# researchaccelerator-hub/distributed-crawler

Measured on AMD Instinct MI355X. Metric: posts/sec (whole node) synthetic feed, higher is better.
Workload: dtype uint8; 1 GPU; model=telegram-crawl 1k-channels x 10k-posts per GPU (BASELINE config #2, weak-scaled), global_batch=1250000, seq_len=0, platform=telegram, parallelism=dp1, channels_per_gpu=1000, posts_per_channel=10000, chunk_posts=1250000, new_discoveries=998486, sink=pinned, pinned=True, max_comments_per_post=3

## Files before the change

crawler_amd/ops/csrc/common.h:

```cpp
#pragma once

#include <hip/hip_runtime.h>
#include <stdint.h>

#define WAVE 64
#define DEV __device__ __forceinline__

typedef unsigned int __attribute__((aligned(1))) u32_unal;
#ifndef CRAWL_NT_STORES
#define CRAWL_NT_STORES 0
#endif
DEV void nt_store_u32(unsigned char* p, unsigned v) {
#if CRAWL_NT_STORES
  __builtin_nontemporal_store(v, (u32_unal*)p);
#else
  __builtin_memcpy(p, &v, 4);
#endif
}
DEV void nt_store_u8(unsigned char* p, unsigned char v) {
#if CRAWL_NT_STORES
  __builtin_nontemporal_store(v, p);
#else
  *p = v;
#endif
}

namespace crawl {

DEV int lane_id() { return threadIdx.x & (WAVE - 1); }
DEV int wave_id() { return threadIdx.x >> 6; }

// ... 220 lines not shown
  DEV void raw(const uint8_t* s, int n) {
    if (W) {
      int lane = lane_id();
      int nw = n >> 2;
      for (int k = lane; k < nw; k += WAVE) {
        unsigned w;
        __builtin_memcpy(&w, s + 4 * k, 4);
        nt_store_u32(out + cur + 4 * k, w);
      }
      for (int j = (nw << 2) + lane; j < n; j += WAVE)
        nt_store_u8(out + cur + j, s[j]);
    }
    cur += n;
  }

  static DEV bool swar_special(unsigned w) {
    unsigned hz;
    unsigned nonascii = w & 0x80808080u;
    unsigned lt20 = (w - 0x20202020u) & ~w & 0x80808080u;
    if (lt20) return true;
    hz = ((w ^ 0x22222222u) - 0x01010101u) & ~(w ^ 0x22222222u);
    hz |= ((w ^ 0x5C5C5C5Cu) - 0x01010101u) & ~(w ^ 0x5C5C5C5Cu);
    hz |= ((w ^ 0x3C3C3C3Cu) - 0x01010101u) & ~(w ^ 0x3C3C3C3Cu);
    hz |= ((w ^ 0x3E3E3E3Eu) - 0x01010101u) & ~(w ^ 0x3E3E3E3Eu);
    hz |= ((w ^ 0x26262626u) - 0x01010101u) & ~(w ^ 0x26262626u);
    if (hz & 0x80808080u) return true;
    if (nonascii) {
      unsigned e2 = ((w ^ 0xE2E2E2E2u) - 0x01010101u) & ~(w ^ 0xE2E2E2E2u);
      if (e2 & 0x80808080u) return true;
    }
// ... 62 lines not shown
        unsigned d;
        if (v <= 0xFFFFFFFFULL)
          d = ((unsigned)v / (unsigned)POW10[lane]) % 10u;
        else
          d = (unsigned)((v / POW10[lane]) % 10ULL);
        nt_store_u8(out + cur + n - 1 - lane, (uint8_t)('0' + d));
      }
    }
    cur += n;
  }
  DEV void i64(long long v) {
    if (v < 0) { LIT(*this, "-"); u64((unsigned long long)(-v)); }
    else u64((unsigned long long)v);
  }

  DEV void rfc3339(long long secs) {
    if (W) rfc3339_write(out, cur, secs);
    cur += 20;
  }
};

DEV uint64_t fnv1a64(const uint8_t* s, int n) {
  uint64_t h = 1469598103934665603ULL;
  for (int i = 0; i < n; ++i) {
    h ^= s[i];
    h *= 1099511628211ULL;
  }
  return h;
}

// ... 2 lines not shown
```

crawler_amd/ops/csrc/parse_encode.hip:

```cpp

#include "common.h"
#include "tg_lits.h"

namespace crawl {

#define MAX_LINKS 8
#define TG_STAGE_BYTES 3968

struct BatchView {
  const long* __restrict__ chat_id;
  const long* __restrict__ msg_id;
  const long* __restrict__ text_off;
  const int* __restrict__ date;
  const int* __restrict__ content_type;
  const int* __restrict__ views;
  const int* __restrict__ forwards;
  const int* __restrict__ media_album_id;
  const int* __restrict__ channel_idx;
  const int* __restrict__ flags;
  const int* __restrict__ text_len;
  const int* __restrict__ aux_off;
  const int* __restrict__ aux_len;
  const int* __restrict__ ent_off;
  const int* __restrict__ ent_cnt;
// ... 24 lines not shown
  const int* __restrict__ ch_title_off;
  const int* __restrict__ ch_title_len;
  const unsigned char* __restrict__ emoji_pool;
  const int* __restrict__ emoji_off;
  const int* __restrict__ emoji_len;
  const unsigned char* __restrict__ created_str;
  int created_len;
  const unsigned char* __restrict__ capture_str;
  int capture_len;
  int n;
  int skip_media;
  long min_post_date;
  const unsigned char* __restrict__ ctname_pool;
  const int* __restrict__ ctname_off;
  const int* __restrict__ ctname_len;
};

struct LinkOut {
  unsigned char* __restrict__ name;
  unsigned char* __restrict__ name_len;
  unsigned char* __restrict__ src;
  int* __restrict__ cnt;
  unsigned long long* __restrict__ hash;
};


DEV void utf16_to_bytes(const unsigned char* s, int n, int off16, int len16,
                        int* out_start, int* out_end) {
  int lane = lane_id();
  int run = 0;
// ... 174 lines not shown
    LIT(*this, "\"");
  }
};

struct StagedTabs {
  const unsigned char* emoji_pool;
  const int* emoji_off;
  const int* emoji_len;
  const unsigned char* created;
  const unsigned char* capture;
  const unsigned char* ctname_pool;
  const int* ctname_off;
  const int* ctname_len;
};

template <bool W, bool STAGED>
DEV int emit_line(const BatchView& B, int i, unsigned char* out,
                  LinkList& L, const unsigned char* lds_lits,
                  unsigned char* lds_stage, const StagedTabs* T) {
  const int lane = lane_id();
  Emit<W> e{};
  e.out = out;
  e.cur = 0;
  e.lds = lds_lits;
  const int c = B.channel_idx[i];
  const unsigned char* user = B.pool + B.ch_user_off[c];
  const int user_n = B.ch_user_len[c];
  const unsigned char* title = B.pool + B.ch_title_off[c];
  const int title_n = B.ch_title_len[c];
  const long pub_id = B.msg_id[i] >> 20;
  const int ct = B.content_type[i];
  const int ncom = B.com_cnt[i];
  const bool has_user = user_n > 0;
  const long chat_id_v = B.chat_id[i];
  const int media_album = B.media_album_id[i];
  const int date_v = B.date[i];
  const int views_v = B.views[i];
  const int forwards_v = B.forwards[i];
  const int ch_member_v = B.ch_member[c];
  const int ch_postcount_v = B.ch_postcount[c];
  const int ch_totalviews_v = B.ch_totalviews[c];
  const int flags_v = B.flags[i];
  const int com0_v = B.com_off[i];
  const int react0_v = B.react_off[i];
// ... 20 lines not shown
  }
  const unsigned char* poster_p = B.pool + poster_off_v;
  const int* re_src = B.react_emoji + react0_v;
  const int* rcnt_src = B.react_count + react0_v;
  const unsigned char* lnames_src = L.names;
  const unsigned char* llens_src = L.lens;
  if (STAGED) {
    int stage_o = 0;
    auto staged = [&](const unsigned char* ptr,
                      int n) -> const unsigned char* {
      unsigned char* dst = lds_stage + stage_o;
      stage_o += n;
      for (int j = lane; j < n; j += WAVE) dst[j] = ptr[j];
      return dst;
    };
    user = staged(user, user_n);
    title = staged(title, title_n);
    poster_p = staged(poster_p, poster_len_v);
    desc_p = staged(desc_p, desc_n);
    lnames_src = staged(L.names, L.cnt * 32);
    llens_src = staged(L.lens, L.cnt);
    stage_o = (stage_o + 3) & ~3;
    int* s_re = (int*)(lds_stage + stage_o);
    stage_o += reactc_v * 4;
    int* s_rc = (int*)(lds_stage + stage_o);
    stage_o += reactc_v * 4;
    for (int j = lane; j < reactc_v; j += WAVE) {
      s_re[j] = B.react_emoji[react0_v + j];
      s_rc[j] = B.react_count[react0_v + j];
    }
    re_src = s_re;
    rcnt_src = s_rc;
  }
  const unsigned char* emoji_pool_s = STAGED ? T->emoji_pool : B.emoji_pool;
  const int* emoji_off_s = STAGED ? T->emoji_off : B.emoji_off;
  const int* emoji_len_s = STAGED ? T->emoji_len : B.emoji_len;
  const unsigned char* created_s = STAGED ? T->created : B.created_str;
  const unsigned char* capture_s = STAGED ? T->capture : B.capture_str;
  const unsigned char* ctpool_s = STAGED ? T->ctname_pool : B.ctname_pool;

  auto post_link = [&]() {
    if (!has_user) { LIT(e, "\"\""); return; }
    TGLIT(e, TGL_0);
    e.esc(user, user_n);
    LIT(e, "/");
    e.i64(pub_id);
    if (media_album != 0) TGLIT(e, TGL_1);
    LIT(e, "\"");
  };

  TGLIT(e, TGL_2);
  post_link();
  TGLIT(e, TGL_3);
  e.i64(chat_id_v);
  TGLIT(e, TGL_4);
  e.i64(pub_id);
  LIT(e, "-");
  e.esc(user, user_n);
  TGLIT(e, TGL_5);
  post_link();
  TGLIT(e, TGL_6);
  e.rfc3339(date_v);
  TGLIT(e, TGL_7);
  e.raw(created_s, B.created_len);
  TGLIT(e, TGL_8);
  e.i64(views_v);
  TGLIT(e, TGL_9);
  e.i64(views_v);
  TGLIT(e, TGL_10);
  e.i64(forwards_v);
  TGLIT(e, TGL_11);
  e.i64(ncom);
  TGLIT(e, TGL_12);
  e.qesc(title, title_n);
  TGLIT(e, TGL_13);
  e.i64(chat_id_v);
  TGLIT(e, TGL_14);
  e.qesc(title, title_n);
  TGLIT(e, TGL_15);
  e.i64(ch_member_v);
  TGLIT(e, TGL_16);
  e.i64(ch_postcount_v);
  TGLIT(e, TGL_17);
  e.i64(ch_totalviews_v);
  TGLIT(e, TGL_18);
  e.esc(user, user_n);
  TGLIT(e, TGL_19);
  e.esc(user, user_n);
  TGLIT(e, TGL_20);
  e.qesc(desc_p, desc_n);
  TGLIT(e, TGL_21);
  e.raw(ctpool_s + (STAGED ? T->ctname_off[ct] : ctname_off_v),
        STAGED ? T->ctname_len[ct] : ctname_len_v);
  TGLIT(e, TGL_22);
  e.i64(forwards_v);
  TGLIT(e, TGL_23);
  e.i64(ncom);
  TGLIT(e, TGL_17);
  e.i64(views_v);
  TGLIT(e, TGL_24);
  TGLIT(e, TGL_25);
  if ((ct == 3 || ct == 8) && (flags_v & 2)) {
    LIT(e, "AgAD");
    e.i64(pub_id);
    LIT(e, "v");
  }
  TGLIT(e, TGL_26);
  {
    const int c0 = com0_v;
    for (int k = 0; k < ncom; ++k) {
      if (k) LIT(e, ",");
      const int cc = c0 + k;
      TGLIT(e, TGL_27);
      e.qesc(B.pool + B.com_text_off[cc], B.com_text_len[cc]);
      TGLIT(e, TGL_28);
      const int r0 = B.com_react_off[cc], rc = B.com_react_cnt[cc];
      for (int r = 0; r < rc; ++r) {
        if (r) LIT(e, ",");
        int em = B.react_emoji[r0 + r];
// ... 27 lines not shown
  for (int k = 0; k < L.cnt; ++k) {
    if (k) LIT(e, ",");
    LIT(e, "\"");
    e.raw(lnames_src + k * 32, llens_src[k]);
    LIT(e, "\"");
  }
  TGLIT(e, TGL_34);
  e.raw(capture_s, B.capture_len);
  TGLIT(e, TGL_35);
  e.qesc(poster_p, poster_len_v);
  LIT(e, "}\n");
  return e.cur;
}


__global__ void __launch_bounds__(256, 6)
measure_extract_kernel(BatchView B, LinkOut LO, int* __restrict__ line_len) {
  __shared__ unsigned char s_lits[TG_POOL_BYTES];
  __shared__ unsigned char s_ln[4][MAX_LINKS * 32];
  __shared__ unsigned char s_ll[4][MAX_LINKS];
  __shared__ unsigned char s_ls[4][MAX_LINKS];
  __shared__ unsigned long long s_lh[4][MAX_LINKS];
  for (int t = threadIdx.x; t < TG_POOL_BYTES; t += blockDim.x)
    s_lits[t] = (unsigned char)tg_lit_pool.v[t];
  __syncthreads();
  const int lane = lane_id();
  const int wave = wave_id();
  const int waves_per_grid = gridDim.x * 4;
  for (int i = blockIdx.x * 4 + wave; i < B.n; i += waves_per_grid) {
    if ((long)B.date[i] < B.min_post_date) {
      if (lane == 0) { line_len[i] = 0; LO.cnt[i] = 0; }
      continue;
    }
    LinkList L{&s_ln[wave][0], &s_ll[wave][0], &s_ls[wave][0],
               &s_lh[wave][0], 0};
    extract_links(B, i, L, lane);
    int len = emit_line<false, false>(B, i, nullptr, L, s_lits,
                                     nullptr, nullptr);
    const int nb = L.cnt * 32;
    unsigned char* gname = LO.name + (size_t)i * MAX_LINKS * 32;
    for (int j = lane; j < nb; j += WAVE) gname[j] = s_ln[wave][j];
    if (lane < L.cnt) {
      LO.name_len[(size_t)i * MAX_LINKS + lane] = s_ll[wave][lane];
      LO.src[(size_t)i * MAX_LINKS + lane] = s_ls[wave][lane];
      LO.hash[(size_t)i * MAX_LINKS + lane] = s_lh[wave][lane];
    }
    if (lane == 0) {
      line_len[i] = len;
      LO.cnt[i] = L.cnt;
    }
  }
}

__global__ void __launch_bounds__(256, 4)
write_kernel(BatchView B, LinkOut LO, const long* __restrict__ line_off,
             const int* __restrict__ line_len, unsigned char* __restrict__ out) {
  __shared__ unsigned char s_lits[TG_POOL_BYTES];
  for (int t = threadIdx.x; t < TG_POOL_BYTES; t += blockDim.x)
    s_lits[t] = (unsigned char)tg_lit_pool.v[t];
  __syncthreads();
  const int lane = lane_id();
  const int wave = wave_id();
  const int waves_per_grid = gridDim.x * 4;
  for (int i = blockIdx.x * 4 + wave; i < B.n; i += waves_per_grid) {
    if (line_len[i] == 0) continue;
    LinkList L{LO.name + (size_t)i * MAX_LINKS * 32,
               LO.name_len + (size_t)i * MAX_LINKS,
               LO.src + (size_t)i * MAX_LINKS,
               LO.hash + (size_t)i * MAX_LINKS, LO.cnt[i]};
    emit_line<true, false>(B, i, out + line_off[i], L, s_lits, nullptr,
                           nullptr);
  }
}

#define TG_EMOJI_POOL_CAP 512
#define TG_EMOJI_CAP 64
#define TG_TS_CAP 64
#define TG_CTNAME_POOL_CAP 512
#define TG_CTNAME_CAP 32

__global__ void __launch_bounds__(256, 4)
write_staged_kernel(BatchView B, LinkOut LO, const long* __restrict__ line_off,
                    const int* __restrict__ line_len,
                    unsigned char* __restrict__ out,
                    int n_emoji, int emoji_pool_bytes,
                    int n_ctnames, int ctname_pool_bytes) {
  __shared__ unsigned char s_lits[TG_POOL_BYTES];
  __shared__ unsigned char s_stage[4][TG_STAGE_BYTES];
  __shared__ unsigned char s_emoji_pool[TG_EMOJI_POOL_CAP];
  __shared__ int s_emoji_off[TG_EMOJI_CAP];
  __shared__ int s_emoji_len[TG_EMOJI_CAP];
  __shared__ unsigned char s_created[TG_TS_CAP];
  __shared__ unsigned char s_capture[TG_TS_CAP];
  __shared__ unsigned char s_ctpool[TG_CTNAME_POOL_CAP];
  __shared__ int s_ctoff[TG_CTNAME_CAP];
  __shared__ int s_ctlen[TG_CTNAME_CAP];
  for (int t = threadIdx.x; t < TG_POOL_BYTES; t += blockDim.x)
    s_lits[t] = (unsigned char)tg_lit_pool.v[t];
  for (int t = threadIdx.x; t < emoji_pool_bytes; t += blockDim.x)
    s_emoji_pool[t] = B.emoji_pool[t];
  for (int t = threadIdx.x; t < n_emoji; t += blockDim.x) {
    s_emoji_off[t] = B.emoji_off[t];
    s_emoji_len[t] = B.emoji_len[t];
// ... 8 lines not shown
    s_ctoff[t] = B.ctname_off[t];
    s_ctlen[t] = B.ctname_len[t];
  }
  __syncthreads();
  StagedTabs T{s_emoji_pool, s_emoji_off, s_emoji_len, s_created,
               s_capture, s_ctpool, s_ctoff, s_ctlen};
  const int lane = lane_id();
  const int wave = wave_id();
  const int waves_per_grid = gridDim.x * 4;
  for (int i = blockIdx.x * 4 + wave; i < B.n; i += waves_per_grid) {
    if (line_len[i] == 0) continue;
    LinkList L{LO.name + (size_t)i * MAX_LINKS * 32,
               LO.name_len + (size_t)i * MAX_LINKS,
               LO.src + (size_t)i * MAX_LINKS,
               LO.hash + (size_t)i * MAX_LINKS, LO.cnt[i]};
    emit_line<true, true>(B, i, out + line_off[i], L, s_lits,
                          &s_stage[wave][0], &T);
  }
}


#define LDS_LINE_BYTES 3072

DEV void copy_line(const unsigned char* src, unsigned char* dst, int n,
                   int lane);

__global__ void __launch_bounds__(256)
write_lds_kernel(BatchView B, LinkOut LO, const long* __restrict__ line_off,
                 const int* __restrict__ line_len, unsigned char* __restrict__ out) {
  __shared__ unsigned char lbuf[4][LDS_LINE_BYTES];
  __shared__ unsigned char s_lits[TG_POOL_BYTES];
  for (int t = threadIdx.x; t < TG_POOL_BYTES; t += blockDim.x)
    s_lits[t] = (unsigned char)tg_lit_pool.v[t];
  __syncthreads();
  const int lane = lane_id();
  const int wave = wave_id();
  const int waves_per_grid = gridDim.x * 4;
  for (int i = blockIdx.x * 4 + wave; i < B.n; i += waves_per_grid) {
    const int len = line_len[i];
    if (len == 0) continue;
    LinkList L{LO.name + (size_t)i * MAX_LINKS * 32,
               LO.name_len + (size_t)i * MAX_LINKS,
               LO.src + (size_t)i * MAX_LINKS,
               LO.hash + (size_t)i * MAX_LINKS, LO.cnt[i]};
    if (len > LDS_LINE_BYTES) {
      emit_line<true, false>(B, i, out + line_off[i], L, s_lits,
                             nullptr, nullptr);
      continue;
    }
    emit_line<true, false>(B, i, &lbuf[wave][0], L, s_lits, nullptr,
                           nullptr);
    copy_line(&lbuf[wave][0], out + line_off[i], len, lane);
  }
}


__global__ void __launch_bounds__(256)
write_scratch_kernel(BatchView B, LinkOut LO, unsigned char* __restrict__ scratch,
                     long stride, int* __restrict__ line_len, int* __restrict__ overflow) {
  __shared__ unsigned char s_lits[TG_POOL_BYTES];
  for (int t = threadIdx.x; t < TG_POOL_BYTES; t += blockDim.x)
    s_lits[t] = (unsigned char)tg_lit_pool.v[t];
  __syncthreads();
  const int lane = lane_id();
  const int wave = wave_id();
  const int waves_per_grid = gridDim.x * 4;
  for (int i = blockIdx.x * 4 + wave; i < B.n; i += waves_per_grid) {
    if ((long)B.date[i] < B.min_post_date) {
      if (lane == 0) { line_len[i] = 0; LO.cnt[i] = 0; }
      continue;
    }
    LinkList L{LO.name + (size_t)i * MAX_LINKS * 32,
               LO.name_len + (size_t)i * MAX_LINKS,
               LO.src + (size_t)i * MAX_LINKS,
               LO.hash + (size_t)i * MAX_LINKS, 0};
    extract_links(B, i, L, lane);
    int len = emit_line<true, false>(B, i, scratch + (size_t)i * stride, L,
                                     s_lits, nullptr, nullptr);
    if (lane == 0) {
      line_len[i] = len;
      LO.cnt[i] = L.cnt;
      if (len > stride) atomicMax(overflow, len);
    }
  }
}

DEV void copy_line(const unsigned char* src, unsigned char* dst, int n,
                   int lane) {
  int h = (int)((4 - ((unsigned long)(size_t)dst & 3)) & 3);
  if (h > n) h = n;
  if (lane == 0)
    for (int j = 0; j < h; ++j) dst[j] = src[j];
  const unsigned char* s = src + h;
// ... 76 lines not shown
  B.ch_member = (const int*)p[k++];
  B.ch_postcount = (const int*)p[k++];
  B.ch_totalviews = (const int*)p[k++];
  B.ch_user_off = (const int*)p[k++];
  B.ch_user_len = (const int*)p[k++];
  B.ch_title_off = (const int*)p[k++];
  B.ch_title_len = (const int*)p[k++];
  B.emoji_pool = (const unsigned char*)p[k++];
  B.emoji_off = (const int*)p[k++];
  B.emoji_len = (const int*)p[k++];
  B.created_str = (const unsigned char*)p[k++];
  B.capture_str = (const unsigned char*)p[k++];
  B.ctname_pool = (const unsigned char*)p[k++];
  B.ctname_off = (const int*)p[k++];
  B.ctname_len = (const int*)p[k++];
  B.n = (int)s[0];
  B.skip_media = (int)s[1];
  B.min_post_date = s[2];
  B.created_len = (int)s[3];
  B.capture_len = (int)s[4];
  return B;
}

static LinkOut make_links(void** p) {
  LinkOut L;
  L.name = (unsigned char*)p[0];
  L.name_len = (unsigned char*)p[1];
  L.src = (unsigned char*)p[2];
  L.cnt = (int*)p[3];
  L.hash = (unsigned long long*)p[4];
  return L;
}

}

extern "C" {

int crawl_batch_ptr_count() { return 49; }

int crawl_measure_extract(void** batch_ptrs, const long* scalars,
                          void** link_ptrs, void* line_len, int grid,
                          void* stream) {
  crawl::BatchView B = crawl::make_view(batch_ptrs, scalars);
  crawl::LinkOut LO = crawl::make_links(link_ptrs);
  hipLaunchKernelGGL(crawl::measure_extract_kernel, dim3(grid), dim3(256), 0,
                     (hipStream_t)stream, B, LO, (int*)line_len);
  return (int)hipGetLastError();
}

int crawl_write(void** batch_ptrs, const long* scalars, void** link_ptrs,
                const void* line_off, const void* line_len, void* out,
                int grid, void* stream) {
  crawl::BatchView B = crawl::make_view(batch_ptrs, scalars);
  crawl::LinkOut LO = crawl::make_links(link_ptrs);
  hipLaunchKernelGGL(crawl::write_kernel, dim3(grid), dim3(256), 0,
                     (hipStream_t)stream, B, LO, (const long*)line_off,
                     (const int*)line_len, (unsigned char*)out);
  return (int)hipGetLastError();
}

int crawl_write_staged(void** batch_ptrs, const long* scalars,
                       void** link_ptrs, const void* line_off,
                       const void* line_len, void* out,
                       int n_emoji, int emoji_pool_bytes,
                       int n_ctnames, int ctname_pool_bytes,
                       int grid, void* stream) {
  crawl::BatchView B = crawl::make_view(batch_ptrs, scalars);
  crawl::LinkOut LO = crawl::make_links(link_ptrs);
  hipLaunchKernelGGL(crawl::write_staged_kernel, dim3(grid), dim3(256), 0,
                     (hipStream_t)stream, B, LO, (const long*)line_off,
                     (const int*)line_len, (unsigned char*)out,
                     n_emoji, emoji_pool_bytes, n_ctnames,
                     ctname_pool_bytes);
  return (int)hipGetLastError();
}

int crawl_stage_budget() { return TG_STAGE_BYTES; }

int crawl_write_scratch(void** batch_ptrs, const long* scalars,
                        void** link_ptrs, void* scratch, long stride,
                        void* line_len, void* overflow, int grid,
                        void* stream) {
  crawl::BatchView B = crawl::make_view(batch_ptrs, scalars);
  crawl::LinkOut LO = crawl::make_links(link_ptrs);
  hipLaunchKernelGGL(crawl::write_scratch_kernel, dim3(grid), dim3(256), 0,
                     (hipStream_t)stream, B, LO, (unsigned char*)scratch,
                     stride, (int*)line_len, (int*)overflow);
  return (int)hipGetLastError();
}

int crawl_write_lds(void** batch_ptrs, const long* scalars, void** link_ptrs,
                    const void* line_off, const void* line_len, void* out,
                    int grid, void* stream) {
  crawl::BatchView B = crawl::make_view(batch_ptrs, scalars);
  crawl::LinkOut LO = crawl::make_links(link_ptrs);
  hipLaunchKernelGGL(crawl::write_lds_kernel, dim3(grid), dim3(256), 0,
                     (hipStream_t)stream, B, LO, (const long*)line_off,
                     (const int*)line_len, (unsigned char*)out);
  return (int)hipGetLastError();
}

int crawl_compact(const void* scratch, long stride, const void* line_off,
                  const void* line_len, void* out, int n, int grid,
                  void* stream) {
  hipLaunchKernelGGL(crawl::compact_kernel, dim3(grid), dim3(256), 0,
                     (hipStream_t)stream, (const unsigned char*)scratch,
                     stride, (const long*)line_off, (const int*)line_len,
                     (unsigned char*)out, n);
  return (int)hipGetLastError();
}

}
```

crawler_amd/ops/gpu.py:

```python
from __future__ import annotations

import ctypes
import dataclasses
import datetime as _dt
import os
from typing import List, Optional, Tuple

import torch

from ..models.post import format_go_time
from . import batch as B

_CSRC = os.path.dirname(os.path.abspath(__file__)) + "/csrc"
_LIB_PATH = os.path.join(_CSRC, "libcrawlhip.so")

MAX_LINKS = 8

_BATCH_PTR_ORDER = [
    "chat_id", "msg_id", "text_off",
    "m:date", "m:content_type", "m:views", "m:forwards", "m:media_album_id",
    "m:channel_idx", "m:flags", "m:text_len", "m:aux_off", "m:aux_len",
    "m:ent_off", "m:ent_cnt", "m:react_off", "m:react_cnt", "m:com_off",
    "m:com_cnt", "m:poster_off", "m:poster_len",
    "text_pool", "entities", "react_emoji", "react_count",
    "com_text_off", "com_text_len", "com_handle_off", "com_handle_len",
    "com_views", "com_replies", "com_react_off", "com_react_cnt",
    "ch_chat_id", "ch_member", "ch_postcount", "ch_totalviews",
    "ch_user_off", "ch_user_len", "ch_title_off", "ch_title_len",
]

_lib = None

_vp_t, _ll, _cl, _ci = (ctypes.c_void_p, ctypes.c_longlong, ctypes.c_long,
                        ctypes.c_int)
_pp = ctypes.POINTER(ctypes.c_void_p)
_lp = ctypes.POINTER(ctypes.c_long)
_SIGNATURES = {
    "crawl_batch_ptr_count": [],
    "crawl_stage_budget": [],
    "crawl_measure_extract": [_pp, _lp, _pp, _vp_t, _ci, _vp_t],
    "crawl_write": [_pp, _lp, _pp, _vp_t, _vp_t, _vp_t, _ci, _vp_t],
    "crawl_write_lds": [_pp, _lp, _pp, _vp_t, _vp_t, _vp_t, _ci, _vp_t],
    "crawl_write_staged": [_pp, _lp, _pp, _vp_t, _vp_t, _vp_t, _ci, _ci,
                           _ci, _ci, _ci, _vp_t],
    "crawl_write_scratch": [_pp, _lp, _pp, _vp_t, _cl, _vp_t, _vp_t, _ci,
                            _vp_t],
    "crawl_compact": [_vp_t, _cl, _vp_t, _vp_t, _vp_t, _ci, _ci, _vp_t],
    "crawl_claim_links": [_vp_t, _vp_t, _ci, _ci, _vp_t, _ll, _vp_t, _vp_t,
                          _ci, _vp_t],
    "crawl_bloom_update": [_vp_t, _vp_t, _ci, _ci, _vp_t, _ll, _ci, _vp_t],
    "crawl_claim_compact": [_vp_t, _vp_t, _vp_t, _vp_t, _ci, _ci, _vp_t,
                            _vp_t, _vp_t, ctypes.c_uint, _ci, _vp_t],
    "crawl_insert_hashes": [_vp_t, _cl, _vp_t, _ll, _ci, _vp_t],
    "crawl_feed_meta": [_pp, _lp, _vp_t, _pp, _ci, _vp_t],
# ... 441 lines not shown


@dataclasses.dataclass
class EncodeResult:

    out: torch.Tensor
    line_off: torch.Tensor
    line_len: torch.Tensor
    link_name: torch.Tensor
    link_len: torch.Tensor
    link_src: torch.Tensor
    link_cnt: torch.Tensor
    link_hash: torch.Tensor
    writer: str = ""
    raw: Optional[torch.Tensor] = None


def _ptr_array(tensors: List[torch.Tensor]):
    arr = (ctypes.c_void_p * len(tensors))()
    for k, t in enumerate(tensors):
        arr[k] = ctypes.c_void_p(t.data_ptr())
    return arr


def _stride_bound(batch: B.MessageBatch) -> int:
    m = batch.meta
    dev = batch.device
    i64 = lambda t: t.to(torch.int64)
    c = m["channel_idx"].to(torch.int64)
    bound = (
        2200
        + 6 * i64(m["text_len"]) + 6 * i64(m["aux_len"])
        + 12 * i64(batch.ch_title_len[c])
        + 36 * i64(batch.ch_user_len[c])
        + 6 * i64(m["poster_len"])
        + 45 * i64(m["react_cnt"])
        + 170 * i64(m["com_cnt"])
        + 35 * MAX_LINKS
    )
    ccnt = i64(m["com_cnt"])
    total_c = int(ccnt.sum().item())
    if total_c:
        extra = (6 * (i64(batch.com_text_len) + i64(batch.com_handle_len))
                 + 45 * i64(batch.com_react_cnt))
        pre = torch.zeros(extra.numel() + 1, dtype=torch.int64, device=dev)
        torch.cumsum(extra, 0, out=pre[1:])
        c0 = i64(m["com_off"])
        bound = bound + pre[c0 + ccnt] - pre[c0]
# ... 123 lines not shown
            tensors.append(batch.meta[name[2:]])
        else:
            tensors.append(getattr(batch, name))
    tensors += [
        tables["emoji_pool"], tables["emoji_off"], tables["emoji_len"],
        created_t, capture_t,
        tables["ctname_pool"], tables["ctname_off"], tables["ctname_len"],
    ]
    names = _BATCH_PTR_ORDER + [
        "emoji_pool", "emoji_off", "emoji_len", "created", "capture",
        "ctname_pool", "ctname_off", "ctname_len",
    ]
    for nm, t in zip(names, tensors):
        assert t.device == dev, f"{nm} on {t.device}, batch on {dev}"
        assert t.is_contiguous(), f"{nm} not contiguous"
    batch_ptrs = _ptr_array(tensors)
    assert len(tensors) == lib.crawl_batch_ptr_count()

    if min_post_date is not None:
        mpd = int(min_post_date.timestamp())
    else:
        mpd = -(1 << 62)
    scalars = (ctypes.c_long * 5)(n, 1, mpd, len(created), len(capture))

    link_name = torch.empty((n, MAX_LINKS, 32), dtype=torch.uint8, device=dev)
    link_len = torch.zeros((n, MAX_LINKS), dtype=torch.uint8, device=dev)
    link_src = torch.zeros((n, MAX_LINKS), dtype=torch.uint8, device=dev)
    link_cnt = torch.zeros(n, dtype=torch.int32, device=dev)
    link_hash = torch.zeros((n, MAX_LINKS), dtype=torch.int64, device=dev)
    line_len = torch.zeros(n, dtype=torch.int32, device=dev)
    link_ptrs = _ptr_array([link_name, link_len, link_src, link_cnt, link_hash])

    if grid <= 0:
        grid = min((n + 3) // 4, 8192)

    stage_need = None
    if (not single_pass and not os.environ.get("CRAWL_LDS_WRITE")
            and os.environ.get("CRAWL_NO_STAGED") != "1"
            and _tables_fit(tables, created, capture)):
        stage_need = _stage_need(batch)
    writer = _pick_writer(os.environ, single_pass, stage_need,
                          _stage_budget(lib))

    if writer == "scratch":
        stride = (_stride_bound(batch) + 31) & ~15
        scratch = torch.empty(n * stride, dtype=torch.uint8, device=dev)
        if _poison is not None:
            scratch.fill_(_poison)
        overflow = torch.zeros(1, dtype=torch.int32, device=dev)
        _call("crawl_write_scratch", batch_ptrs, scalars, link_ptrs, scratch,
              stride, line_len, overflow, grid, stream=stream)
        line_off = torch.zeros(n, dtype=torch.int64, device=dev)
        torch.cumsum(line_len.to(torch.int64)[:-1], 0, out=line_off[1:])
        total = int(line_off[-1].item() + line_len[-1].item()) if n else 0
        ovf = int(overflow.item())
        if ovf:
            raise RuntimeError(
                f"line overflowed scratch stride ({ovf} > {stride}); "
                "stride bound is unsound for this batch"
            )
        out, raw = _alloc_out(total, dev, _poison, _guard)
        _call("crawl_compact", scratch, stride, line_off, line_len, out, n,
              grid, stream=stream)
    else:
        _call("crawl_measure_extract", batch_ptrs, scalars, link_ptrs,
              line_len, grid, stream=stream)
        line_off = torch.zeros(n, dtype=torch.int64, device=dev)
        torch.cumsum(line_len.to(torch.int64)[:-1], 0, out=line_off[1:])
        total = int(line_off[-1].item() + line_len[-1].item()) if n else 0
        out, raw = _alloc_out(total, dev, _poison, _guard)
        if writer == "staged":
            _call("crawl_write_staged", batch_ptrs, scalars, link_ptrs,
                  line_off, line_len, out, tables["emoji_off"].numel(),
                  tables["emoji_pool"].numel(), tables["ctname_off"].numel(),
                  tables["ctname_pool"].numel(), grid, stream=stream)
        else:
            _call("crawl_write_lds" if writer == "lds" else "crawl_write",
                  batch_ptrs, scalars, link_ptrs, line_off, line_len, out,
                  grid, stream=stream)

    return EncodeResult(
        out=out, line_off=line_off, line_len=line_len,
        link_name=link_name, link_len=link_len, link_src=link_src,
        link_cnt=link_cnt, link_hash=link_hash, writer=writer, raw=raw,
    )


class SeenSet:

    def __init__(self, device, slots_log2: int = 22, bloom_bits_log2: int = 26):
        self.device = device
        self.slots = 1 << slots_log2
        self.bloom_bits = 1 << bloom_bits_log2
        self.table = torch.zeros(self.slots, dtype=torch.int64, device=device)
        self.bloom = torch.zeros(
            self.bloom_bits // 32, dtype=torch.int32, device=device
        )
        self._n_new = torch.zeros(1, dtype=torch.int32, device=device)
        self.lib = require_lib()
# ... 83 lines not shown
```

Baseline: 27.74 million posts/s.

## Pre-render per-channel constant JSON runs once and splice them into post lines

Adds a chan_consts kernel that renders each channel's invariant JSON fragments (escaped title, member/postcount/views, names, post-link prefix) once into 16-byte-aligned rows. The measure and write kernels then copy these runs with 128-bit stores, staging them in LDS when they fit, instead of re-escaping and re-formatting the same channel strings for every post. It also computes the decimal digits of repeated integers once per line and reuses them. In exchange it adds an extra kernel launch, per-channel row buffers, extra LDS in the staged writer and a host sync to check for row overflow.

```diff
diff --git a/crawler_amd/ops/csrc/common.h b/crawler_amd/ops/csrc/common.h
--- a/crawler_amd/ops/csrc/common.h
+++ b/crawler_amd/ops/csrc/common.h
@@ -15,6 +15,15 @@
   __builtin_nontemporal_store(v, (u32_unal*)p);
 #else
   __builtin_memcpy(p, &v, 4);
+#endif
+}
+typedef unsigned int u32x4 __attribute__((ext_vector_type(4)));
+typedef u32x4 __attribute__((aligned(1))) u32x4_unal;
+DEV void nt_store_u128(unsigned char* p, u32x4 v) {
+#if CRAWL_NT_STORES
+  __builtin_nontemporal_store(v, (u32x4_unal*)p);
+#else
+  *(u32x4_unal*)p = v;
 #endif
 }
 DEV void nt_store_u8(unsigned char* p, unsigned char v) {
@@ -265,6 +274,20 @@
     cur += n;
   }
 
+  DEV void wide(const uint8_t* s, int n) {
+    if (W) {
+      int lane = lane_id();
+      int nq = n >> 4;
+      for (int k = lane; k < nq; k += WAVE) {
+        u32x4 q = *(const u32x4*)(s + 16 * k);
+        nt_store_u128(out + cur + 16 * k, q);
+      }
+      for (int j = (nq << 4) + lane; j < n; j += WAVE)
+        nt_store_u8(out + cur + j, s[j]);
+    }
+    cur += n;
+  }
+
   static DEV bool swar_special(unsigned w) {
     unsigned hz;
     unsigned nonascii = w & 0x80808080u;
@@ -357,6 +380,44 @@
     else u64((unsigned long long)v);
   }
 
+  struct Dec {
+    int n;
+  };
+  DEV Dec dec_prep(long long v, unsigned* chars, int slot) {
+    static const unsigned long long POW10[20] = {
+        1ULL, 10ULL, 100ULL, 1000ULL, 10000ULL, 100000ULL, 1000000ULL,
+        10000000ULL, 100000000ULL, 1000000000ULL, 10000000000ULL,
+        100000000000ULL, 1000000000000ULL, 10000000000000ULL,
+        100000000000000ULL, 1000000000000000ULL, 10000000000000000ULL,
+        100000000000000000ULL, 1000000000000000000ULL,
+        10000000000000000000ULL};
+    const bool neg = v < 0;
+    const unsigned long long u =
+        neg ? (unsigned long long)(-v) : (unsigned long long)v;
+    const int nd = u64_dec_len(u);
+    if (W) {
+      int lane = lane_id();
+      unsigned ch = '-';
+      if (lane < nd) {
+        if (u <= 0xFFFFFFFFULL)
+          ch = '0' + ((unsigned)u / (unsigned)POW10[lane]) % 10u;
+        else
+          ch = '0' + (unsigned)((u / POW10[lane]) % 10ULL);
+      }
+      *chars |= ch << (8 * slot);
+    }
+    return Dec{nd + (neg ? 1 : 0)};
+  }
+  DEV void dec(Dec d, unsigned chars, int slot) {
+    if (W) {
+      int lane = lane_id();
+      if (lane < d.n)
+        nt_store_u8(out + cur + d.n - 1 - lane,
+                    (uint8_t)(chars >> (8 * slot)));
+    }
+    cur += d.n;
+  }
+
   DEV void rfc3339(long long secs) {
     if (W) rfc3339_write(out, cur, secs);
     cur += 20;
diff --git a/crawler_amd/ops/csrc/parse_encode.hip b/crawler_amd/ops/csrc/parse_encode.hip
--- a/crawler_amd/ops/csrc/parse_encode.hip
+++ b/crawler_amd/ops/csrc/parse_encode.hip
@@ -62,6 +62,10 @@
   const unsigned char* __restrict__ ctname_pool;
   const int* __restrict__ ctname_off;
   const int* __restrict__ ctname_len;
+  const unsigned char* __restrict__ cc_rows;
+  const int* __restrict__ cc_meta;
+  int n_channels;
+  long cc_stride;
 };
 
 struct LinkOut {
@@ -266,20 +270,127 @@
   const int* ctname_len;
 };
 
-template <bool W, bool STAGED>
+enum { CC_LEN_A, CC_LEN_B, CC_LEN_P, CC_LEN_U, CC_OFF_B, CC_OFF_P, CC_OFF_U,
+       CC_USER_N, CC_META };
+#define TG_CC_LDS_BYTES 2048
+
+struct ChanRuns {
+  int len_a, len_b, len_p, len_u, off_b, off_p, off_u;
+  DEV int total() const { return off_u + len_u; }
+};
+
+DEV int cc_align(int v) { return (v + 15) & ~15; }
+
+template <bool W>
+DEV ChanRuns render_chan_runs(const BatchView& B, int c, unsigned char* row,
+                              const unsigned char* lds_lits) {
+  const unsigned char* user = B.pool + B.ch_user_off[c];
+  const int user_n = B.ch_user_len[c];
+  const unsigned char* title = B.pool + B.ch_title_off[c];
+  const int title_n = B.ch_title_len[c];
+  const int member = B.ch_member[c];
+  const int postcount = B.ch_postcount[c];
+  const int totalviews = B.ch_totalviews[c];
+  const unsigned char* name = user_n > 0 ? user : title;
+  const int name_n = user_n > 0 ? user_n : title_n;
+  ChanRuns R;
+  Emit<W> e{};
+  e.out = row;
+  e.cur = 0;
+  e.lds = lds_lits;
+  TGLIT(e, TGL_12);
+  e.qesc(title, title_n);
+  TGLIT(e, TGL_13);
+  R.len_a = e.cur;
+  R.off_b = e.cur = cc_align(e.cur);
+  TGLIT(e, TGL_14);
+  e.qesc(title, title_n);
+  TGLIT(e, TGL_15);
+  e.i64(member);
+  TGLIT(e, TGL_16);
+  e.i64(postcount);
+  TGLIT(e, TGL_17);
+  e.i64(totalviews);
+  TGLIT(e, TGL_18);
+  e.esc(name, name_n);
+  TGLIT(e, TGL_19);
+  e.esc(name, name_n);
+  TGLIT(e, TGL_20);
+  R.len_b = e.cur - R.off_b;
+  R.off_p = e.cur = cc_align(e.cur);
+  if (user_n > 0) {
+    TGLIT(e, TGL_0);
+    e.esc(user, user_n);
+    LIT(e, "/");
+  } else {
+    LIT(e, "\"\"");
+  }
+  R.len_p = e.cur - R.off_p;
+  R.off_u = e.cur = cc_align(e.cur);
+  LIT(e, "-");
+  e.esc(name, name_n);
+  TGLIT(e, TGL_5);
+  R.len_u = e.cur - R.off_u;
+  return R;
+}
+
+__global__ void __launch_bounds__(256)
+chan_consts_kernel(BatchView B, unsigned char* __restrict__ rows,
+                   int* __restrict__ meta, int* __restrict__ err) {
+  __shared__ unsigned char s_lits[TG_POOL_BYTES];
+  for (int t = threadIdx.x; t < TG_POOL_BYTES; t += blockDim.x)
+    s_lits[t] = (unsigned char)tg_lit_pool.v[t];
+  __syncthreads();
+  const int c = blockIdx.x * 4 + wave_id();
+  if (c >= B.n_channels) return;
+  ChanRuns R = render_chan_runs<false>(B, c, nullptr, s_lits);
+  const bool fits = (long)cc_align(R.total()) <= B.cc_stride;
+  if (fits)
+    render_chan_runs<true>(B, c, rows + (size_t)c * B.cc_stride, s_lits);
+  if (lane_id() == 0) {
+    int* m = meta + (size_t)c * CC_META;
+    m[CC_LEN_A] = fits ? R.len_a : 0;
+    m[CC_LEN_B] = fits ? R.len_b : 0;
+    m[CC_LEN_P] = fits ? R.len_p : 0;
+    m[CC_LEN_U] = fits ? R.len_u : 0;
+    m[CC_OFF_B] = fits ? R.off_b : 0;
+    m[CC_OFF_P] = fits ? R.off_p : 0;
+    m[CC_OFF_U] = fits ? R.off_u : 0;
+    m[CC_USER_N] = B.ch_user_len[c];
+    if (!fits) atomicMax(err, R.total());
+  }
+}
+
+template <bool W, bool STAGED, bool FOLD>
 DEV int emit_line(const BatchView& B, int i, unsigned char* out,
                   LinkList& L, const unsigned char* lds_lits,
-                  unsigned char* lds_stage, const StagedTabs* T) {
+                  unsigned char* lds_stage, const StagedTabs* T,
+                  unsigned char* lds_cc) {
   const int lane = lane_id();
   Emit<W> e{};
   e.out = out;
   e.cur = 0;
   e.lds = lds_lits;
   const int c = B.channel_idx[i];
-  const unsigned char* user = B.pool + B.ch_user_off[c];
-  const int user_n = B.ch_user_len[c];
-  const unsigned char* title = B.pool + B.ch_title_off[c];
-  const int title_n = B.ch_title_len[c];
+  const unsigned char* user = nullptr;
+  int user_n = 0;
+  const unsigned char* title = nullptr;
+  int title_n = 0;
+  ChanRuns R{};
+  const unsigned char* cc_row = nullptr;
+  if (FOLD) {
+    const int4* mp = (const int4*)(B.cc_meta + (size_t)c * CC_META);
+    const int4 m0 = mp[0], m1 = mp[1];
+    R.len_a = m0.x; R.len_b = m0.y; R.len_p = m0.z; R.len_u = m0.w;
+    R.off_b = m1.x; R.off_p = m1.y; R.off_u = m1.z;
+    user_n = m1.w;
+    cc_row = B.cc_rows + (size_t)c * B.cc_stride;
+  } else {
+    user = B.pool + B.ch_user_off[c];
+    user_n = B.ch_user_len[c];
+    title = B.pool + B.ch_title_off[c];
+    title_n = B.ch_title_len[c];
+  }
   const long pub_id = B.msg_id[i] >> 20;
   const int ct = B.content_type[i];
   const int ncom = B.com_cnt[i];
@@ -330,8 +441,10 @@
       for (int j = lane; j < n; j += WAVE) dst[j] = ptr[j];
       return dst;
     };
-    user = staged(user, user_n);
-    title = staged(title, title_n);
+    if (!FOLD) {
+      user = staged(user, user_n);
+      title = staged(title, title_n);
+    }
     poster_p = staged(poster_p, poster_len_v);
     desc_p = staged(desc_p, desc_n);
     lnames_src = staged(L.names, L.cnt * 32);
@@ -355,12 +468,45 @@
   const unsigned char* capture_s = STAGED ? T->capture : B.capture_str;
   const unsigned char* ctpool_s = STAGED ? T->ctname_pool : B.ctname_pool;
 
+  unsigned dch0 = 0, dch1 = 0;
+  const auto d_pub = e.dec_prep(pub_id, &dch0, 0);
+  const auto d_chat = e.dec_prep(chat_id_v, &dch0, 1);
+  const auto d_views = e.dec_prep(views_v, &dch0, 2);
+  const auto d_fwd = e.dec_prep(forwards_v, &dch0, 3);
+  const auto d_ncom = e.dec_prep(ncom, &dch1, 0);
+  auto emit_pub = [&]() { e.dec(d_pub, dch0, 0); };
+  auto emit_chat = [&]() { e.dec(d_chat, dch0, 1); };
+  auto emit_views = [&]() { e.dec(d_views, dch0, 2); };
+  auto emit_fwd = [&]() { e.dec(d_fwd, dch0, 3); };
+  auto emit_ncom = [&]() { e.dec(d_ncom, dch1, 0); };
+
+  bool cc_in_lds = false;
+  if (W && STAGED && FOLD) {
+    const int total = R.total();
+    cc_in_lds = total <= TG_CC_LDS_BYTES;
+    if (cc_in_lds)
+      for (int j = 16 * lane; j < total; j += 16 * WAVE)
+        *(u32x4*)(lds_cc + j) = *(const u32x4*)(cc_row + j);
+  }
+  auto cc_run = [&](int off, int n) {
+    if (STAGED && cc_in_lds) e.wide(lds_cc + off, n);
+    else e.wide(cc_row + off, n);
+  };
+
+  const unsigned char* name = has_user ? user : title;
+  const int name_n = has_user ? user_n : title_n;
+
   auto post_link = [&]() {
-    if (!has_user) { LIT(e, "\"\""); return; }
-    TGLIT(e, TGL_0);
-    e.esc(user, user_n);
-    LIT(e, "/");
-    e.i64(pub_id);
+    if (FOLD) {
+      cc_run(R.off_p, R.len_p);
+      if (!has_user) return;
+    } else {
+      if (!has_user) { LIT(e, "\"\""); return; }
+      TGLIT(e, TGL_0);
+      e.esc(user, user_n);
+      LIT(e, "/");
+    }
+    emit_pub();
     if (media_album != 0) TGLIT(e, TGL_1);
     LIT(e, "\"");
   };
@@ -368,57 +514,67 @@
   TGLIT(e, TGL_2);
   post_link();
   TGLIT(e, TGL_3);
-  e.i64(chat_id_v);
+  emit_chat();
   TGLIT(e, TGL_4);
-  e.i64(pub_id);
-  LIT(e, "-");
-  e.esc(user, user_n);
-  TGLIT(e, TGL_5);
+  emit_pub();
+  if (FOLD) {
+    cc_run(R.off_u, R.len_u);
+  } else {
+    LIT(e, "-");
+    e.esc(name, name_n);
+    TGLIT(e, TGL_5);
+  }
   post_link();
   TGLIT(e, TGL_6);
   e.rfc3339(date_v);
   TGLIT(e, TGL_7);
   e.raw(created_s, B.created_len);
   TGLIT(e, TGL_8);
-  e.i64(views_v);
+  emit_views();
   TGLIT(e, TGL_9);
-  e.i64(views_v);
+  emit_views();
   TGLIT(e, TGL_10);
-  e.i64(forwards_v);
+  emit_fwd();
   TGLIT(e, TGL_11);
-  e.i64(ncom);
-  TGLIT(e, TGL_12);
-  e.qesc(title, title_n);
-  TGLIT(e, TGL_13);
-  e.i64(chat_id_v);
-  TGLIT(e, TGL_14);
-  e.qesc(title, title_n);
-  TGLIT(e, TGL_15);
-  e.i64(ch_member_v);
-  TGLIT(e, TGL_16);
-  e.i64(ch_postcount_v);
-  TGLIT(e, TGL_17);
-  e.i64(ch_totalviews_v);
-  TGLIT(e, TGL_18);
-  e.esc(user, user_n);
-  TGLIT(e, TGL_19);
-  e.esc(user, user_n);
-  TGLIT(e, TGL_20);
+  emit_ncom();
+  if (FOLD) {
+    cc_run(0, R.len_a);
+    emit_chat();
+    cc_run(R.off_b, R.len_b);
+  } else {
+    TGLIT(e, TGL_12);
+    e.qesc(title, title_n);
+    TGLIT(e, TGL_13);
+    emit_chat();
+    TGLIT(e, TGL_14);
+    e.qesc(title, title_n);
+    TGLIT(e, TGL_15);
+    e.i64(ch_member_v);
+    TGLIT(e, TGL_16);
+    e.i64(ch_postcount_v);
+    TGLIT(e, TGL_17);
+    e.i64(ch_totalviews_v);
+    TGLIT(e, TGL_18);
+    e.esc(name, name_n);
+    TGLIT(e, TGL_19);
+    e.esc(name, name_n);
+    TGLIT(e, TGL_20);
+  }
   e.qesc(desc_p, desc_n);
   TGLIT(e, TGL_21);
   e.raw(ctpool_s + (STAGED ? T->ctname_off[ct] : ctname_off_v),
         STAGED ? T->ctname_len[ct] : ctname_len_v);
   TGLIT(e, TGL_22);
-  e.i64(forwards_v);
+  emit_fwd();
   TGLIT(e, TGL_23);
-  e.i64(ncom);
+  emit_ncom();
   TGLIT(e, TGL_17);
-  e.i64(views_v);
+  emit_views();
   TGLIT(e, TGL_24);
   TGLIT(e, TGL_25);
   if ((ct == 3 || ct == 8) && (flags_v & 2)) {
     LIT(e, "AgAD");
-    e.i64(pub_id);
+    emit_pub();
     LIT(e, "v");
   }
   TGLIT(e, TGL_26);
@@ -476,6 +632,7 @@
 }
 
 
+template <bool FOLD>
 __global__ void __launch_bounds__(256, 6)
 measure_extract_kernel(BatchView B, LinkOut LO, int* __restrict__ line_len) {
   __shared__ unsigned char s_lits[TG_POOL_BYTES];
@@ -497,8 +654,8 @@
     LinkList L{&s_ln[wave][0], &s_ll[wave][0], &s_ls[wave][0],
                &s_lh[wave][0], 0};
     extract_links(B, i, L, lane);
-    int len = emit_line<false, false>(B, i, nullptr, L, s_lits,
-                                     nullptr, nullptr);
+    int len = emit_line<false, false, FOLD>(B, i, nullptr, L, s_lits,
+                                           nullptr, nullptr, nullptr);
     const int nb = L.cnt * 32;
     unsigned char* gname = LO.name + (size_t)i * MAX_LINKS * 32;
     for (int j = lane; j < nb; j += WAVE) gname[j] = s_ln[wave][j];
@@ -514,6 +671,7 @@
   }
 }
 
+template <bool FOLD>
 __global__ void __launch_bounds__(256, 4)
 write_kernel(BatchView B, LinkOut LO, const long* __restrict__ line_off,
              const int* __restrict__ line_len, unsigned char* __restrict__ out) {
@@ -530,8 +688,8 @@
                LO.name_len + (size_t)i * MAX_LINKS,
                LO.src + (size_t)i * MAX_LINKS,
                LO.hash + (size_t)i * MAX_LINKS, LO.cnt[i]};
-    emit_line<true, false>(B, i, out + line_off[i], L, s_lits, nullptr,
-                           nullptr);
+    emit_line<true, false, FOLD>(B, i, out + line_off[i], L, s_lits,
+                                 nullptr, nullptr, nullptr);
   }
 }
 
@@ -541,6 +699,7 @@
 #define TG_CTNAME_POOL_CAP 512
 #define TG_CTNAME_CAP 32
 
+template <bool FOLD>
 __global__ void __launch_bounds__(256, 4)
 write_staged_kernel(BatchView B, LinkOut LO, const long* __restrict__ line_off,
                     const int* __restrict__ line_len,
@@ -549,6 +708,8 @@
                     int n_ctnames, int ctname_pool_bytes) {
   __shared__ unsigned char s_lits[TG_POOL_BYTES];
   __shared__ unsigned char s_stage[4][TG_STAGE_BYTES];
+  __shared__ __attribute__((aligned(16)))
+  unsigned char s_cc[FOLD ? 4 : 1][FOLD ? TG_CC_LDS_BYTES : 16];
   __shared__ unsigned char s_emoji_pool[TG_EMOJI_POOL_CAP];
   __shared__ int s_emoji_off[TG_EMOJI_CAP];
   __shared__ int s_emoji_len[TG_EMOJI_CAP];
@@ -587,8 +748,8 @@
                LO.name_len + (size_t)i * MAX_LINKS,
                LO.src + (size_t)i * MAX_LINKS,
                LO.hash + (size_t)i * MAX_LINKS, LO.cnt[i]};
-    emit_line<true, true>(B, i, out + line_off[i], L, s_lits,
-                          &s_stage[wave][0], &T);
+    emit_line<true, true, FOLD>(B, i, out + line_off[i], L, s_lits,
+                                &s_stage[wave][0], &T, &s_cc[wave][0]);
   }
 }
 
@@ -598,6 +759,7 @@
 DEV void copy_line(const unsigned char* src, unsigned char* dst, int n,
                    int lane);
 
+template <bool FOLD>
 __global__ void __launch_bounds__(256)
 write_lds_kernel(BatchView B, LinkOut LO, const long* __restrict__ line_off,
                  const int* __restrict__ line_len, unsigned char* __restrict__ out) {
@@ -617,17 +779,18 @@
                LO.src + (size_t)i * MAX_LINKS,
                LO.hash + (size_t)i * MAX_LINKS, LO.cnt[i]};
     if (len > LDS_LINE_BYTES) {
-      emit_line<true, false>(B, i, out + line_off[i], L, s_lits,
-                             nullptr, nullptr);
+      emit_line<true, false, FOLD>(B, i, out + line_off[i], L, s_lits,
+                                   nullptr, nullptr, nullptr);
       continue;
     }
-    emit_line<true, false>(B, i, &lbuf[wave][0], L, s_lits, nullptr,
-                           nullptr);
+    emit_line<true, false, FOLD>(B, i, &lbuf[wave][0], L, s_lits, nullptr,
+                                 nullptr, nullptr);
     copy_line(&lbuf[wave][0], out + line_off[i], len, lane);
   }
 }
 
 
+template <bool FOLD>
 __global__ void __launch_bounds__(256)
 write_scratch_kernel(BatchView B, LinkOut LO, unsigned char* __restrict__ scratch,
                      long stride, int* __restrict__ line_len, int* __restrict__ overflow) {
@@ -648,8 +811,9 @@
                LO.src + (size_t)i * MAX_LINKS,
                LO.hash + (size_t)i * MAX_LINKS, 0};
     extract_links(B, i, L, lane);
-    int len = emit_line<true, false>(B, i, scratch + (size_t)i * stride, L,
-                                     s_lits, nullptr, nullptr);
+    int len = emit_line<true, false, FOLD>(
+        B, i, scratch + (size_t)i * stride, L, s_lits, nullptr, nullptr,
+        nullptr);
     if (lane == 0) {
       line_len[i] = len;
       LO.cnt[i] = L.cnt;
@@ -756,11 +920,15 @@
   B.ctname_pool = (const unsigned char*)p[k++];
   B.ctname_off = (const int*)p[k++];
   B.ctname_len = (const int*)p[k++];
+  B.cc_rows = (const unsigned char*)p[k++];
+  B.cc_meta = (const int*)p[k++];
   B.n = (int)s[0];
   B.skip_media = (int)s[1];
   B.min_post_date = s[2];
   B.created_len = (int)s[3];
   B.capture_len = (int)s[4];
+  B.n_channels = (int)s[5];
+  B.cc_stride = s[6];
   return B;
 }
 
@@ -778,15 +946,35 @@
 
 extern "C" {
 
-int crawl_batch_ptr_count() { return 49; }
+int crawl_batch_ptr_count() { return 51; }
+
+#define CRAWL_LAUNCH_FOLD(kernel, B, ...)                              \
+  do {                                                                 \
+    if ((B).cc_rows)                                                   \
+      hipLaunchKernelGGL(crawl::kernel<true>, dim3(grid), dim3(256),   \
+                         0, (hipStream_t)stream, __VA_ARGS__);         \
+    else                                                               \
+      hipLaunchKernelGGL(crawl::kernel<false>, dim3(grid), dim3(256),  \
+                         0, (hipStream_t)stream, __VA_ARGS__);         \
+  } while (0)
+
+int crawl_chan_consts(void** batch_ptrs, const long* scalars, void* err,
+                      void* stream) {
+  crawl::BatchView B = crawl::make_view(batch_ptrs, scalars);
+  if (B.n_channels <= 0) return 0;
+  hipLaunchKernelGGL(crawl::chan_consts_kernel,
+                     dim3((B.n_channels + 3) / 4), dim3(256), 0,
+                     (hipStream_t)stream, B, (unsigned char*)B.cc_rows,
+                     (int*)B.cc_meta, (int*)err);
+  return (int)hipGetLastError();
+}
 
 int crawl_measure_extract(void** batch_ptrs, const long* scalars,
                           void** link_ptrs, void* line_len, int grid,
                           void* stream) {
   crawl::BatchView B = crawl::make_view(batch_ptrs, scalars);
   crawl::LinkOut LO = crawl::make_links(link_ptrs);
-  hipLaunchKernelGGL(crawl::measure_extract_kernel, dim3(grid), dim3(256), 0,
-                     (hipStream_t)stream, B, LO, (int*)line_len);
+  CRAWL_LAUNCH_FOLD(measure_extract_kernel, B, B, LO, (int*)line_len);
   return (int)hipGetLastError();
 }
 
@@ -795,9 +983,8 @@
                 int grid, void* stream) {
   crawl::BatchView B = crawl::make_view(batch_ptrs, scalars);
   crawl::LinkOut LO = crawl::make_links(link_ptrs);
-  hipLaunchKernelGGL(crawl::write_kernel, dim3(grid), dim3(256), 0,
-                     (hipStream_t)stream, B, LO, (const long*)line_off,
-                     (const int*)line_len, (unsigned char*)out);
+  CRAWL_LAUNCH_FOLD(write_kernel, B, B, LO, (const long*)line_off,
+                    (const int*)line_len, (unsigned char*)out);
   return (int)hipGetLastError();
 }
 
@@ -809,11 +996,9 @@
                        int grid, void* stream) {
   crawl::BatchView B = crawl::make_view(batch_ptrs, scalars);
   crawl::LinkOut LO = crawl::make_links(link_ptrs);
-  hipLaunchKernelGGL(crawl::write_staged_kernel, dim3(grid), dim3(256), 0,
-                     (hipStream_t)stream, B, LO, (const long*)line_off,
-                     (const int*)line_len, (unsigned char*)out,
-                     n_emoji, emoji_pool_bytes, n_ctnames,
-                     ctname_pool_bytes);
+  CRAWL_LAUNCH_FOLD(write_staged_kernel, B, B, LO, (const long*)line_off,
+                    (const int*)line_len, (unsigned char*)out, n_emoji,
+                    emoji_pool_bytes, n_ctnames, ctname_pool_bytes);
   return (int)hipGetLastError();
 }
 
@@ -825,9 +1010,8 @@
                         void* stream) {
   crawl::BatchView B = crawl::make_view(batch_ptrs, scalars);
   crawl::LinkOut LO = crawl::make_links(link_ptrs);
-  hipLaunchKernelGGL(crawl::write_scratch_kernel, dim3(grid), dim3(256), 0,
-                     (hipStream_t)stream, B, LO, (unsigned char*)scratch,
-                     stride, (int*)line_len, (int*)overflow);
+  CRAWL_LAUNCH_FOLD(write_scratch_kernel, B, B, LO, (unsigned char*)scratch,
+                    stride, (int*)line_len, (int*)overflow);
   return (int)hipGetLastError();
 }
 
@@ -836,9 +1020,8 @@
                     int grid, void* stream) {
   crawl::BatchView B = crawl::make_view(batch_ptrs, scalars);
   crawl::LinkOut LO = crawl::make_links(link_ptrs);
-  hipLaunchKernelGGL(crawl::write_lds_kernel, dim3(grid), dim3(256), 0,
-                     (hipStream_t)stream, B, LO, (const long*)line_off,
-                     (const int*)line_len, (unsigned char*)out);
+  CRAWL_LAUNCH_FOLD(write_lds_kernel, B, B, LO, (const long*)line_off,
+                    (const int*)line_len, (unsigned char*)out);
   return (int)hipGetLastError();
 }
 
diff --git a/crawler_amd/ops/gpu.py b/crawler_amd/ops/gpu.py
--- a/crawler_amd/ops/gpu.py
+++ b/crawler_amd/ops/gpu.py
@@ -38,6 +38,7 @@
 _SIGNATURES = {
     "crawl_batch_ptr_count": [],
     "crawl_stage_budget": [],
+    "crawl_chan_consts": [_pp, _lp, _vp_t, _vp_t],
     "crawl_measure_extract": [_pp, _lp, _pp, _vp_t, _ci, _vp_t],
     "crawl_write": [_pp, _lp, _pp, _vp_t, _vp_t, _vp_t, _ci, _vp_t],
     "crawl_write_lds": [_pp, _lp, _pp, _vp_t, _vp_t, _vp_t, _ci, _vp_t],
@@ -509,13 +510,58 @@
     link_hash: torch.Tensor
     writer: str = ""
     raw: Optional[torch.Tensor] = None
-
-
-def _ptr_array(tensors: List[torch.Tensor]):
+    folded: bool = False
+
+
+def _ptr_array(tensors: List[Optional[torch.Tensor]]):
     arr = (ctypes.c_void_p * len(tensors))()
     for k, t in enumerate(tensors):
-        arr[k] = ctypes.c_void_p(t.data_ptr())
+        arr[k] = ctypes.c_void_p(None if t is None else t.data_ptr())
     return arr
+
+
+_CC_FIXED_A = 49 + 330 + 2
+_CC_FIXED_B = 615 + 2 + 3 * 11
+_CC_FIXED_P = 14 + 1
+_CC_FIXED_U = 1 + 8
+_CC_META = 8
+_CC_MIN_POSTS_PER_CHANNEL = 1
+
+
+def _align16(v: int) -> int:
+    return (v + 15) & ~15
+
+
+def _chan_run_bounds(title_len: int, user_len: int):
+    t, u = 6 * title_len, 6 * user_len
+    name = max(u, t)
+    return (_CC_FIXED_A + t, _CC_FIXED_B + t + 2 * name,
+            max(_CC_FIXED_P + u, 2), _CC_FIXED_U + name)
+
+
+def _chan_row_stride(max_title_len: int, max_user_len: int) -> int:
+    return sum(_align16(b) for b in
+               _chan_run_bounds(max_title_len, max_user_len))
+
+
+def _chan_max_lens(batch) -> Tuple[int, int]:
+    got = getattr(batch, "_chan_max_lens", None)
+    if got is None:
+        got = tuple(int(v) for v in torch.stack(
+            [batch.ch_title_len.max(), batch.ch_user_len.max()]).tolist())
+        try:
+            batch._chan_max_lens = got
+        except AttributeError:
+            pass
+    return got
+
+
+def _fold_channels(n: int, n_channels: int) -> bool:
+    if n_channels <= 0 or os.environ.get("CRAWL_NO_CHAN_FOLD") == "1":
+        return False
+    if os.environ.get("CRAWL_CHAN_FOLD") == "1":
+        return True
+    return n >= _CC_MIN_POSTS_PER_CHANNEL * n_channels
 
 
 def _stride_bound(batch: B.MessageBatch) -> int:
@@ -526,7 +572,7 @@
     bound = (
         2200
         + 6 * i64(m["text_len"]) + 6 * i64(m["aux_len"])
-        + 12 * i64(batch.ch_title_len[c])
+        + 30 * i64(batch.ch_title_len[c])
         + 36 * i64(batch.ch_user_len[c])
         + 6 * i64(m["poster_len"])
         + 45 * i64(m["react_cnt"])
@@ -680,6 +726,17 @@
     for nm, t in zip(names, tensors):
         assert t.device == dev, f"{nm} on {t.device}, batch on {dev}"
         assert t.is_contiguous(), f"{nm} not contiguous"
+    fold = _fold_channels(n, batch.n_channels)
+    cc_rows = cc_meta = cc_err = None
+    cc_stride = 0
+    if fold:
+        cc_stride = _chan_row_stride(*_chan_max_lens(batch))
+        cc_rows = torch.empty(batch.n_channels * cc_stride,
+                              dtype=torch.uint8, device=dev)
+        cc_meta = torch.empty(batch.n_channels * _CC_META,
+                              dtype=torch.int32, device=dev)
+        cc_err = torch.zeros(1, dtype=torch.int32, device=dev)
+    tensors += [cc_rows, cc_meta]
     batch_ptrs = _ptr_array(tensors)
     assert len(tensors) == lib.crawl_batch_ptr_count()
 
@@ -687,7 +744,8 @@
         mpd = int(min_post_date.timestamp())
     else:
         mpd = -(1 << 62)
-    scalars = (ctypes.c_long * 5)(n, 1, mpd, len(created), len(capture))
+    scalars = (ctypes.c_long * 7)(n, 1, mpd, len(created), len(capture),
+                                  batch.n_channels, cc_stride)
 
     link_name = torch.empty((n, MAX_LINKS, 32), dtype=torch.uint8, device=dev)
     link_len = torch.zeros((n, MAX_LINKS), dtype=torch.uint8, device=dev)
@@ -707,6 +765,16 @@
         stage_need = _stage_need(batch)
     writer = _pick_writer(os.environ, single_pass, stage_need,
                           _stage_budget(lib))
+
+    def check_rows():
+        if fold and int(cc_err.item()):
+            raise RuntimeError(
+                f"a channel's runs ({int(cc_err.item())} bytes) exceed the "
+                f"row stride {cc_stride}; the stride bound is unsound")
+
+    if fold:
+        _call("crawl_chan_consts", batch_ptrs, scalars, cc_err,
+              stream=stream)
 
     if writer == "scratch":
         stride = (_stride_bound(batch) + 31) & ~15
@@ -719,6 +787,7 @@
         line_off = torch.zeros(n, dtype=torch.int64, device=dev)
         torch.cumsum(line_len.to(torch.int64)[:-1], 0, out=line_off[1:])
         total = int(line_off[-1].item() + line_len[-1].item()) if n else 0
+        check_rows()
         ovf = int(overflow.item())
         if ovf:
             raise RuntimeError(
@@ -734,6 +803,7 @@
         line_off = torch.zeros(n, dtype=torch.int64, device=dev)
         torch.cumsum(line_len.to(torch.int64)[:-1], 0, out=line_off[1:])
         total = int(line_off[-1].item() + line_len[-1].item()) if n else 0
+        check_rows()
         out, raw = _alloc_out(total, dev, _poison, _guard)
         if writer == "staged":
             _call("crawl_write_staged", batch_ptrs, scalars, link_ptrs,
@@ -749,6 +819,7 @@
         out=out, line_off=line_off, line_len=line_len,
         link_name=link_name, link_len=link_len, link_src=link_src,
         link_cnt=link_cnt, link_hash=link_hash, writer=writer, raw=raw,
+        folded=fold,
     )
 
 
```

Measured after the change: 27.93 million posts/s (median of 5 runs). About the same (+0.7%).
